# IntptrMax/YoloSharp

Measured on AMD Instinct MI355X. Metric: train images/sec YOLOv8n 640x640 bs=64/GPU, higher is better.
Workload: dtype bf16; 1 GPU; YOLOv8n detect train step (fwd+loss+bwd+AdamW), 64x3x640x640 per GPU, COCO-80 synthetic labels; global_batch=64, parallelism=dp1

## Files before the change

yolosharp_amd/csrc/conv_wgrad.hip:

```cpp
#include "ys_internal.h"
#include "ys_kernels.h"
#include <atomic>
#include <cstdlib>

template <class T, int MRA, int NRB>
__global__ void __launch_bounds__(256)
conv_wgrad_kernel(WgradArgs a) {
  constexpr int EPL = Elem<T>::EPL;
  constexpr int KS = 4 * EPL;
  constexpr int COT = MRA * 16, CIT = NRB * 16;
  constexpr int PD = COT + 16 / (int)sizeof(T);
  constexpr int PX = CIT + 16 / (int)sizeof(T);
  constexpr int STAGE_BYTES = 4 * KS * (PD + PX) * (int)sizeof(T);
  constexpr int RED_BYTES = 4 * COT * CIT * 4;
  constexpr int LDS_BYTES = STAGE_BYTES > RED_BYTES ? STAGE_BYTES : RED_BYTES;
  __shared__ uint4 smem[LDS_BYTES / 16];
  T* sD = (T*)smem;
  T* sX = sD + 4 * KS * PD;

  const int tid = threadIdx.x, lane = tid & 63, wave = tid >> 6, li = lane & 15, q = lane >> 4;
  const int ci_tiles = (a.Cin + CIT - 1) / CIT;
  const int co0 = (blockIdx.y / ci_tiles) * COT;
  const int ci0 = (blockIdx.y % ci_tiles) * CIT;
  const int tap = blockIdx.z;
  const int kh = tap / a.KW, kw = tap % a.KW;
  const int HWo = a.Hout * a.Wout;
  const long steps_total = ((long)a.M + KS - 1) / KS;
  const long steps_per_blk = (steps_total + gridDim.x - 1) / gridDim.x;
  const long sb = (long)blockIdx.x * steps_per_blk;
  long se = sb + steps_per_blk;
  if (se > steps_total) se = steps_total;
  const long iters = (steps_per_blk + 3) / 4;

  f32x4 acc[MRA][NRB];
#pragma unroll
  for (int i = 0; i < MRA; i++)
#pragma unroll
    for (int j = 0; j < NRB; j++) acc[i][j] = f32x4_zero();

  T* myD = sD + wave * KS * PD;
  T* myX = sX + wave * KS * PX;
  const char* dyb = (const char*)a.dy;
  const char* xb = (const char*)a.x;
  constexpr int DV = COT / EPL;
  constexpr int XV = CIT / EPL;

  constexpr int ND = (KS * DV + 63) / 64, NX = (KS * XV + 63) / 64;
  uint4 rd[ND], rx[NX];
  auto fetch = [&](long it) {
    const long step = sb + it * 4 + wave;
    const bool active = step < se;
    const long p0 = step * KS;
#pragma unroll
    for (int k = 0; k < ND; k++) {
      const int v = lane + 64 * k;
      const int pr = v / DV, cv = v % DV;
      const long p = p0 + pr;
      const int c = co0 + cv * EPL;
      uint4 val = ys_zero16();
      if (v < KS * DV && active && p < a.M && c < a.Cout) {
        const long bb = p / HWo;
        const long rr = p - bb * HWo;
        const long drow = a.dy_rh ? bb * a.dy_bstride + (rr / a.Wout) * a.dy_rh + (rr % a.Wout) * a.dy_rw + a.dy_r0
                                  : bb * a.dy_bstride + rr;
        val = ys_ld16(dyb + ((drow * a.dy_ldc) + a.dy_coff + c) * (long)sizeof(T));
      }
      rd[k] = val;
    }
#pragma unroll
    for (int k = 0; k < NX; k++) {
      const int v = lane + 64 * k;
      const int pr = v / XV, cv = v % XV;
      const long p = p0 + pr;
      const int c = ci0 + cv * EPL;
      uint4 val = ys_zero16();
      if (v < KS * XV && active && p < a.M && c < a.Cin) {
        const int b = (int)(p / HWo);
        const int r = (int)(p - (long)b * HWo);
        const int oh = r / a.Wout, ow = r - oh * a.Wout;
        const int ih = oh * a.stride + kh - a.pad, iw = ow * a.stride + kw - a.pad;
        if (ih >= 0 && ih < a.Hin && iw >= 0 && iw < a.Win)
          val = ys_ld16(xb + ((((long)b * a.in_bstride + (long)ih * a.Win + iw) * a.in_ldc) + a.in_coff + c) * (long)sizeof(T));
      }
      rx[k] = val;
    }
  };
  fetch(0);
  for (long it = 0; it < iters; it++) {
#pragma unroll
    for (int k = 0; k < ND; k++) {
      const int v = lane + 64 * k;
      if (v < KS * DV) *(uint4*)(myD + (v / DV) * PD + (v % DV) * EPL) = rd[k];
    }
#pragma unroll
    for (int k = 0; k < NX; k++) {
      const int v = lane + 64 * k;
      if (v < KS * XV) *(uint4*)(myX + (v / XV) * PX + (v % XV) * EPL) = rx[k];
    }
    ys_wave_sync();
    if (it + 1 < iters) fetch(it + 1);
    uint4 fa[MRA], fb[NRB];
#pragma unroll
    for (int i = 0; i < MRA; i++) {
      alignas(16) T tmp[EPL];
#pragma unroll
      for (int e = 0; e < EPL; e++) tmp[e] = myD[(q * EPL + e) * PD + i * 16 + li];
      fa[i] = ys_pack_elems(tmp);
    }
#pragma unroll
    for (int j = 0; j < NRB; j++) {
      alignas(16) T tmp[EPL];
#pragma unroll
      for (int e = 0; e < EPL; e++) tmp[e] = myX[(q * EPL + e) * PX + j * 16 + li];
      fb[j] = ys_pack_elems(tmp);
    }
#pragma unroll
    for (int i = 0; i < MRA; i++)
#pragma unroll
      for (int j = 0; j < NRB; j++) acc[i][j] = ys_mma<T>(fa[i], fb[j], acc[i][j]);
    ys_wave_sync();
  }
  __syncthreads();
  float* sR = (float*)smem;
#pragma unroll
  for (int i = 0; i < MRA; i++)
#pragma unroll
    for (int j = 0; j < NRB; j++)
#pragma unroll
      for (int r = 0; r < 4; r++)
        sR[(wave * COT + i * 16 + 4 * q + r) * CIT + j * 16 + li] = acc[i][j][r];
  __syncthreads();
  float* outp = a.partial + (long)blockIdx.x * a.Cout * a.KH * a.KW * a.Cin;
  for (int e = tid; e < COT * CIT; e += 256) {
    const int co = co0 + e / CIT, ci = ci0 + e % CIT;
    if (co < a.Cout && ci < a.Cin) {
      const float v = sR[e] + sR[COT * CIT + e] + sR[2 * COT * CIT + e] + sR[3 * COT * CIT + e];
      outp[((long)co * a.KH * a.KW + tap) * a.Cin + ci] = v;
    }
  }
}

__global__ void __launch_bounds__(512)
wgrad_reduce_kernel(const float* __restrict__ partial, int splits, long n, int cin_pad, int cin_real,
                    float* __restrict__ grad) {
  __shared__ float sred[16][32];
  const int o = threadIdx.x & 31, sl = threadIdx.x >> 5;
  const long i = (long)blockIdx.x * 32 + o;
  float gprev = 0.f; long gidx = -1;
  if (sl == 0 && i < n) {
    const long row = i / cin_pad;
    const int ci = (int)(i - row * cin_pad);
    if (ci < cin_real) { gidx = row * cin_real + ci; gprev = grad[gidx]; }
  }
  float s0 = 0.f, s1 = 0.f, s2 = 0.f, s3 = 0.f;
  if (i < n) {
    int k = sl;
    for (; k + 48 < splits; k += 64) {
      s0 += partial[(long)k * n + i];
      s1 += partial[(long)(k + 16) * n + i];
      s2 += partial[(long)(k + 32) * n + i];
      s3 += partial[(long)(k + 48) * n + i];
    }
    for (; k < splits; k += 16) s0 += partial[(long)k * n + i];
  }
  sred[sl][o] = (s0 + s1) + (s2 + s3);
  __syncthreads();
  if (gidx >= 0) {
    float t = 0.f;
#pragma unroll
    for (int w = 0; w < 16; w++) t += sred[w][o];
    grad[gidx] = gprev + t;
  }
}

__device__ __forceinline__ unsigned wg_uniform(unsigned v) {
#ifdef YS_EMU_BUILD
  return v;
#else
  return (unsigned)__builtin_amdgcn_readfirstlane((int)v);
#endif
}
#define YS_WG_TWO_MAX 2
template <int MRA, int NRB, int TAPS>
__global__ void __launch_bounds__(TAPS == 9 ? 576 : 256, (TAPS == 9 && MRA * NRB <= YS_WG_TWO_MAX) ? 5 : 1)
conv_wgrad_tr_kernel(WgradArgs a) {
  constexpr int NT = TAPS == 9 ? 576 : 256;
  constexpr int NW = NT / 64;
  constexpr int COT = MRA * 16, CIT = NRB * 16;
  constexpr int DV = COT / 8, XV = CIT / 8;
  constexpr int TPMAX = TAPS == 9 ? 256 : 128;
  constexpr int ND = (TPMAX * DV + NT - 1) / NT;
  constexpr int NX = TAPS == 9 ? 5 : (TPMAX * XV + NT - 1) / NT;
  YS_DYN_LDS(lds);
  const int tid = threadIdx.x, lane = tid & 63, wave = tid >> 6, li = lane & 15, q = lane >> 4;
  const int TW = 1 << a.TWS, TP = a.TH * TW;
  const int nkb = (TP + 31) >> 5;
  const int ZR = nkb * 32;
  char* sDb = (char*)lds;
  const int ci_tiles = (a.Cin + CIT - 1) / CIT;
  const int co0 = (blockIdx.y / ci_tiles) * COT;
  const int ci0 = (blockIdx.y % ci_tiles) * CIT;
  const char* dyb = (const char*)a.dy;
  const char* xb = (const char*)a.x;
  const int S = a.stride;
  const int npatch = a.PH * a.PW * XV;

  for (int i = tid; i < a.pdb / 4; i += NT) ((unsigned*)(sDb + (size_t)ZR * a.pdb))[i] = 0u;

  const ys_rsrcv_t rsD = ys_make_rsrcv(dyb + (long)a.dy_coff * 2L, a.dybytes);
  const ys_rsrcv_t rsX = ys_make_rsrcv(xb + (long)a.in_coff * 2L, a.xbytes);
  uint4 rd[ND], rx[NX];
  constexpr unsigned YS_WG_NOUNIT = 0xffffffffu;
  unsigned doff[ND], drc[ND], dlds[ND], xoff[NX], xrc[NX], xlds[NX];
#pragma unroll
  for (int k = 0; k < ND; k++) {
    const int idx = tid + NT * k;
    const int p = idx / DV, u = idx - p * DV;
    const int ty = p >> a.TWS, tx = p & (TW - 1);
    const int c = co0 + u * 8;
    const bool slot = idx < TP * DV;
    doff[k] = (((unsigned)ty * (unsigned)a.Wout + (unsigned)tx) * (unsigned)a.dy_ldc + (unsigned)c) * 2u;
    drc[k] = (slot && c < a.Cout) ? ((unsigned)ty << 16 | (unsigned)tx) : YS_WG_NOUNIT;
    dlds[k] = slot ? (unsigned)(p * a.pdb + u * 16) : YS_WG_NOUNIT;
#ifndef YS_EMU_BUILD
    asm volatile("" : "+v"(doff[k]), "+v"(drc[k]), "+v"(dlds[k]));
#endif
  }
#pragma unroll
  for (int k = 0; k < NX; k++) {
    const int idx = tid + NT * k;
    const int pix = idx / XV, u = idx - pix * XV;
    const int r = pix / a.PW, cc = pix - r * a.PW;
    const int c = ci0 + u * 8;
    const bool slot = idx < npatch;
    xoff[k] = (((unsigned)r * (unsigned)a.Win + (unsigned)cc) * (unsigned)a.in_ldc + (unsigned)c) * 2u;
    xrc[k] = (slot && c < a.Cin) ? ((unsigned)r << 16 | (unsigned)cc) : YS_WG_NOUNIT;
    xlds[k] = slot ? (unsigned)((ZR + 1) * a.pdb + pix * a.pxb + u * 16) : YS_WG_NOUNIT;
#ifndef YS_EMU_BUILD
    asm volatile("" : "+v"(xoff[k]), "+v"(xrc[k]), "+v"(xlds[k]));
#endif
  }
  auto fetch = [&](int txi, int tyi, int b) {
    const int oy0 = tyi * a.TH, ox0 = txi * TW;
    const unsigned dh = (unsigned)((a.Hout - oy0) < a.TH ? (a.Hout - oy0) : a.TH), dw = (unsigned)((a.Wout - ox0) < TW ? (a.Wout - ox0) : TW);
    const unsigned dorg = wg_uniform((((unsigned)b * (unsigned)a.dy_bstride + (unsigned)oy0 * (unsigned)a.Wout + (unsigned)ox0) * (unsigned)a.dy_ldc) * 2u);
#pragma unroll
    for (int k = 0; k < ND; k++) {
      const bool ok = (bool)((int)((drc[k] >> 16) < dh) & (int)((drc[k] & 0xffffu) < dw));
      rd[k] = ys_bufld16(rsD, ok ? dorg + doff[k] : YS_BUF_OOB);
    }
    const int iy0 = oy0 * S - a.pad, ix0 = ox0 * S - a.pad;
    const unsigned rlo = iy0 < 0 ? (unsigned)-iy0 : 0u, clo = ix0 < 0 ? (unsigned)-ix0 : 0u;
    const unsigned rn = (unsigned)((a.Hin - iy0) < a.PH ? (a.Hin - iy0) : a.PH) - rlo, cn = (unsigned)((a.Win - ix0) < a.PW ? (a.Win - ix0) : a.PW) - clo;
    const unsigned xorg = wg_uniform((((unsigned)b * (unsigned)a.in_bstride + (unsigned)iy0 * (unsigned)a.Win + (unsigned)ix0) * (unsigned)a.in_ldc) * 2u);
#pragma unroll
    for (int k = 0; k < NX; k++) {
      const bool ok = (bool)((int)(((xrc[k] >> 16) - rlo) < rn) & (int)(((xrc[k] & 0xffffu) - clo) < cn));
      rx[k] = ys_bufld16(rsX, ok ? xorg + xoff[k] : YS_BUF_OOB);
    }
  };
  int stx, sty, stb;
  {
    const int G = (int)gridDim.x;
    stx = G % a.tiles_x; const int rem = G / a.tiles_x;
    sty = rem % a.tiles_y; stb = rem / a.tiles_y;
  }
  auto advance = [&](int& txi, int& tyi, int& b) {
    txi += stx; if (txi >= a.tiles_x) { txi -= a.tiles_x; tyi++; }
    tyi += sty; if (tyi >= a.tiles_y) { tyi -= a.tiles_y; b++; }
    b += stb;
  };

  f32x4 acc[MRA][NRB];
#pragma unroll
  for (int i = 0; i < MRA; i++)
#pragma unroll
    for (int j = 0; j < NRB; j++) acc[i][j] = f32x4_zero();

  const int tap = TAPS == 9 ? wave : 0;
  const int kh = tap / 3, kw = tap - kh * 3;
  const int rr = li >> 2, c4 = li & 3;
  unsigned dof[2], xof[2];
  int ty0[2], tx0[2];
#pragma unroll
  for (int h = 0; h < 2; h++) {
    const int p0 = 16 * h + 4 * q + rr;
    ty0[h] = p0 >> a.TWS; tx0[h] = p0 & (TW - 1);
    dof[h] = (unsigned)(p0 * a.pdb + c4 * 8);
    xof[h] = (unsigned)((size_t)(ZR + 1) * a.pdb) + (unsigned)(((ty0[h] * S + kh) * a.PW + tx0[h] * S + kw) * a.pxb + c4 * 8);
  }
  const unsigned dstep = 32u * (unsigned)a.pdb;
  const unsigned xstep = (unsigned)((32 >> a.TWS) * S * a.PW * a.pxb);
  const unsigned zof = (unsigned)(ZR * a.pdb + c4 * 8);
  const unsigned xzero = (unsigned)((ZR + 1) * a.pdb + c4 * 8);
  const int rows_kb = 32 >> a.TWS;
  const char* lb = (const char*)lds;

  int tile = blockIdx.x;
  int txi, tyi, b;
  {
    int t = tile;
    txi = t % a.tiles_x; t /= a.tiles_x;
    tyi = t % a.tiles_y; b = t / a.tiles_y;
  }
  int ntx = txi, nty = tyi, nb = b;
  if (tile < a.ntiles) fetch(txi, tyi, b);
  while (tile < a.ntiles) {
    ys_barrier_lds();
#pragma unroll
    for (int k = 0; k < ND; k++)
      if (dlds[k] != YS_WG_NOUNIT) *(uint4*)((char*)lds + dlds[k]) = rd[k];
#pragma unroll
    for (int k = 0; k < NX; k++)
      if (xlds[k] != YS_WG_NOUNIT) *(uint4*)((char*)lds + xlds[k]) = rx[k];
    ys_barrier_lds();
    const int oy0 = tyi * a.TH, ox0 = txi * TW;
    const int ntile = tile + gridDim.x;
    advance(ntx, nty, nb);
    if (ntile < a.ntiles) fetch(ntx, nty, nb);
    const int tylim = (a.Hout - oy0) < a.TH ? (a.Hout - oy0) : a.TH;
    const bool colok0 = (ox0 + tx0[0]) < a.Wout, colok1 = (ox0 + tx0[1]) < a.Wout;
    for (int kb = (TAPS == 9 ? 0 : wave); kb < nkb; kb += (TAPS == 9 ? 1 : NW)) {
      uint2 ra[2][MRA], rb[2][NRB];
#pragma unroll
      for (int h = 0; h < 2; h++) {
        const int ty = ty0[h] + kb * rows_kb;
        const bool ok = (h == 0 ? colok0 : colok1) && ty < tylim;
        const unsigned d = ok ? dof[h] + (unsigned)kb * dstep : zof;
        const unsigned x = ty < a.TH ? xof[h] + (unsigned)kb * xstep : xzero;
#pragma unroll
        for (int i = 0; i < MRA; i++) ra[h][i] = ys_lds_tr_b64(lb + d + i * 32);
#pragma unroll
        for (int j = 0; j < NRB; j++) rb[h][j] = ys_lds_tr_b64(lb + x + j * 32);
      }
#pragma unroll
      for (int i = 0; i < MRA; i++) ys_lds_tr_wait(ra[0][i], ra[1][i]);
#pragma unroll
      for (int j = 0; j < NRB; j++) ys_lds_tr_wait(rb[0][j], rb[1][j]);
      uint4 fa[MRA], fb[NRB];
#pragma unroll
      for (int i = 0; i < MRA; i++) fa[i] = make_uint4(ra[0][i].x, ra[0][i].y, ra[1][i].x, ra[1][i].y);
#pragma unroll
      for (int j = 0; j < NRB; j++) fb[j] = make_uint4(rb[0][j].x, rb[0][j].y, rb[1][j].x, rb[1][j].y);
#pragma unroll
      for (int i = 0; i < MRA; i++)
#pragma unroll
        for (int j = 0; j < NRB; j++) acc[i][j] = ys_mma<bf16_t>(fa[i], fb[j], acc[i][j]);
    }
    tile = ntile; txi = ntx; tyi = nty;
  }

  float* outp = a.partial + (long)blockIdx.x * a.Cout * a.KH * a.KW * a.Cin;
  const int taps = a.KH * a.KW;
  if (TAPS == 9) {
#pragma unroll
    for (int i = 0; i < MRA; i++)
#pragma unroll
      for (int j = 0; j < NRB; j++)
#pragma unroll
        for (int r = 0; r < 4; r++) {
          const int co = co0 + i * 16 + 4 * q + r, ci = ci0 + j * 16 + li;
          if (co < a.Cout && ci < a.Cin) outp[((long)co * taps + tap) * a.Cin + ci] = acc[i][j][r];
        }
  } else {
    __syncthreads();
    float* sR = (float*)lds;
#pragma unroll
    for (int i = 0; i < MRA; i++)
#pragma unroll
      for (int j = 0; j < NRB; j++)
#pragma unroll
        for (int r = 0; r < 4; r++) sR[(wave * COT + i * 16 + 4 * q + r) * CIT + j * 16 + li] = acc[i][j][r];
    __syncthreads();
    for (int e = tid; e < COT * CIT; e += NT) {
      const int co = co0 + e / CIT, ci = ci0 + e % CIT;
      if (co < a.Cout && ci < a.Cin) {
        float v = 0.f;
        for (int w = 0; w < NW; w++) v += sR[w * COT * CIT + e];
        outp[(long)co * a.Cin + ci] = v;
      }
    }
  }
}

struct WgPlan { int ok, taps9, mra, nrb, th, tws, tx, ty, ph, pw, pdb, pxb, gx; size_t lds; };
static int wg_pitch_bytes(int ch) {
  int s = (ch * 2 + 31) / 32;
  if (!(s & 1)) s++;
  return s * 32;
}
static bool wgrad_view_bytes(const WgradArgs& a, unsigned& dyb, unsigned& xb) {
  const long dpix = (long)(a.B - 1) * a.dy_bstride + (long)a.Hout * a.Wout, xpix = (long)(a.B - 1) * a.in_bstride + (long)a.Hin * a.Win;
  const long d = (dpix * a.dy_ldc - a.dy_coff) * 2L, x = (xpix * a.in_ldc - a.in_coff) * 2L;
  if (d <= 0 || x <= 0 || d >= (1L << 31) || x >= (1L << 31)) return false;
  dyb = (unsigned)d; xb = (unsigned)x;
  return true;
}
#ifdef YS_TRIAGE
static int g_wg_force_th = 0, g_wg_force_tws = 0, g_wg_force_percu = 0;
extern "C" __attribute__((visibility("default"))) int ys_debug_wgrad_force(int th, int tws, int per_cu) { g_wg_force_th = th; g_wg_force_tws = tws; g_wg_force_percu = per_cu; return 0; }
#else
constexpr int g_wg_force_th = 0, g_wg_force_tws = 0, g_wg_force_percu = 0;
#endif
static WgPlan wgrad_tr_plan(const WgradArgs& a) {
  WgPlan p{};
  { unsigned d0, x0; if (!wgrad_view_bytes(a, d0, x0)) return p; }
  const bool k3 = a.KH == 3 && a.KW == 3 && a.pad == 1 && (a.stride == 1 || a.stride == 2);
  const bool k1 = a.KH == 1 && a.KW == 1 && a.pad == 0 && a.stride == 1;
  if (a.dy_rh || !(k3 || k1)) return p;
  const int cof = (a.Cout + 15) / 16, cif = (a.Cin + 15) / 16;
  p.mra = cof >= 4 ? ((cof % 5 == 0) ? 5 : 4) : cof;
  p.nrb = cif >= 4 ? 4 : cif;
  p.taps9 = k3 ? 1 : 0;
  if (k3) {
    static const int ok_pairs[][2] = {{1, 1}, {1, 2}, {1, 3}, {1, 4}, {2, 1}, {2, 2}, {2, 3}, {2, 4}, {3, 1}, {3, 2}, {3, 3}, {3, 4}, {4, 1}, {4, 2}, {5, 1}};
    int best_cost = 1 << 30;
    for (auto& pr : ok_pairs) {
      const int m = pr[0], n = pr[1];
      if (m > cof || n > cif) continue;
      const int cost = ys_cdiv(cof, m) * ys_cdiv(cif, n) * (m + n) * 16 + (ys_cdiv(cof, m) * m - cof) + (ys_cdiv(cif, n) * n - cif) + (n > m ? 1 : 0);
      if (cost < best_cost) { best_cost = cost; p.mra = m; p.nrb = n; }
    }
  }
  const int nt = k3 ? 576 : 256, tpmax = k3 ? 256 : 128;
  const int cot = p.mra * 16, cit = p.nrb * 16, xv = cit / 8;
  const int nxu = (k3 ? 5 : (tpmax * xv + nt - 1) / nt) * nt;
  const int S = a.stride;
  p.pdb = wg_pitch_bytes(cot);
  p.pxb = S == 1 ? wg_pitch_bytes(cit) : ((cit * 2 + 15) / 32) * 32 + 16;
  double best = 1e30;
  for (int tws = 2; tws <= 5; tws++) {
    const int tw = 1 << tws;
    if (tw > a.Wout && tws > 2 && (tw >> 1) >= a.Wout) continue;
    if (g_wg_force_tws && tws != g_wg_force_tws) continue;
    for (int th = 1; th <= a.Hout && th * tw <= tpmax; th++) {
      if (g_wg_force_th && th != g_wg_force_th) continue;
      const int ph = (th - 1) * S + a.KH, pw = (tw - 1) * S + a.KW;
      if (ph * pw * xv > nxu) continue;
      const int nkb = (th * tw + 31) / 32;
      size_t lds = (size_t)(nkb * 32 + 1) * p.pdb + (size_t)ph * pw * p.pxb;
      if (!k3 && lds < (size_t)4 * cot * cit * 4) lds = (size_t)4 * cot * cit * 4;
      if (lds > 150 * 1024) continue;
      const int tx = ys_cdiv(a.Wout, tw), ty = ys_cdiv(a.Hout, th);
      const double cost = (double)tx * ty * ((double)ph * pw * cit + (double)nkb * 32 * cot + 0.5 * nkb * 32 * (cot + cit) + 3000.0);
      if (cost < best) { best = cost; p.ok = 1; p.th = th; p.tws = tws; p.tx = tx; p.ty = ty; p.ph = ph; p.pw = pw; p.lds = lds; }
    }
  }
  if (!p.ok) return p;
  const int gy = ys_cdiv(a.Cout, cot) * ys_cdiv(a.Cin, cit);
  const long ntiles = (long)p.tx * p.ty * a.B;
  int per_cu = (int)((150 * 1024) / p.lds);
  const int per_cu_max = k3 ? (p.mra * p.nrb <= YS_WG_TWO_MAX ? 2 : 1) : 4;
  if (per_cu > per_cu_max) per_cu = per_cu_max;
  if (g_wg_force_percu && g_wg_force_percu < per_cu) per_cu = g_wg_force_percu;
  if (per_cu < 1) per_cu = 1;
  long gx = ((long)ys_cu_count() * per_cu) / gy;
  gx = gx / 8 * 8;
  if (gx < 8) gx = 8;
  const long wsmax = (48L << 20) / ((long)a.Cout * a.KH * a.KW * a.Cin * 4);
  if (gx > wsmax) gx = wsmax > 0 ? wsmax : 1;
  if (gx > ntiles) gx = ntiles;
  const long per = (ntiles + gx - 1) / gx;
  gx = (ntiles + per - 1) / per;
  p.gx = (int)gx;
  return p;
}

template <int MRA, int NRB, int TAPS>
static void wgrad_tr_launch_t(hipStream_t st, WgradArgs a, const WgPlan& p) {
  a.TH = p.th; a.TWS = p.tws; a.tiles_x = p.tx; a.tiles_y = p.ty; a.ntiles = p.tx * p.ty * a.B;
  wgrad_view_bytes(a, a.dybytes, a.xbytes);
  a.PH = p.ph; a.PW = p.pw; a.pdb = p.pdb; a.pxb = p.pxb;
  const int gy = ys_cdiv(a.Cout, MRA * 16) * ys_cdiv(a.Cin, NRB * 16);
  static std::atomic<unsigned> attr_done{0};
  int dev_id = 0;
  (void)hipGetDevice(&dev_id);
  if (!(attr_done.load(std::memory_order_relaxed) & (1u << (dev_id & 31)))) {
    hipFuncSetAttribute((const void*)conv_wgrad_tr_kernel<MRA, NRB, TAPS>, hipFuncAttributeMaxDynamicSharedMemorySize, 160 * 1024);
    attr_done.fetch_or(1u << (dev_id & 31), std::memory_order_relaxed);
  }
  char lab[160] = "";
  if (ys_kprof_enabled()) snprintf(lab, sizeof(lab), "wgrad_tr k%d s%d cin%d cout%d M%d tile%dx%d grid%dx%d lds%d", a.KH, a.stride, a.Cin, a.Cout, a.M, p.th, 1 << p.tws, p.gx, gy, (int)p.lds);
  YsKprofScope prof(st, "conv_wgrad", lab);
  YS_LAUNCH_LDS((conv_wgrad_tr_kernel<MRA, NRB, TAPS>), dim3(p.gx, gy), (TAPS == 9 ? 576 : 256), p.lds, st, a);
}

static bool wgrad_tr_dispatch(hipStream_t st, const WgradArgs& a, const WgPlan& p) {
#define WT(M_, N_) if (p.mra == M_ && p.nrb == N_) { if (p.taps9) wgrad_tr_launch_t<M_, N_, 9>(st, a, p); else wgrad_tr_launch_t<M_, N_, 1>(st, a, p); return true; }
  WT(1, 1) WT(1, 2) WT(1, 3) WT(1, 4)
  WT(2, 1) WT(2, 2) WT(2, 3) WT(2, 4)
  WT(3, 1) WT(3, 2) WT(3, 3) WT(3, 4)
  WT(4, 1) WT(4, 2) WT(4, 3) WT(4, 4)
  WT(5, 1) WT(5, 2) WT(5, 3) WT(5, 4)
#undef WT
  return false;
}

template <class T, int MRA, int NRB>
static void wgrad_launch_t(hipStream_t st, const WgradArgs& a, int splits) {
  const int co_tiles = ys_cdiv(a.Cout, MRA * 16), ci_tiles = ys_cdiv(a.Cin, NRB * 16);
  dim3 grid(splits, co_tiles * ci_tiles, a.KH * a.KW);
  char lab[128] = "";
  if (ys_kprof_enabled()) snprintf(lab, sizeof(lab), "wgrad k%d s%d cin%d cout%d M%d splits%d tiles%d", a.KH, a.stride, a.Cin, a.Cout, a.M, splits, co_tiles * ci_tiles);
  YsKprofScope prof(st, "conv_wgrad", lab);
  YS_LAUNCH((conv_wgrad_kernel<T, MRA, NRB>), grid, 256, st, a);
}

template <class T>
static void wgrad_dispatch(hipStream_t st, const WgradArgs& a, int splits) {
  const int cof = (a.Cout + 15) / 16, cif = (a.Cin + 15) / 16;
  const int mra = cof >= 4 ? ((cof % 5 == 0) ? 5 : 4) : cof;
  const int nrb = cif >= 4 ? 4 : cif;
#define WG(M_, N_) if (mra == M_ && nrb == N_) { wgrad_launch_t<T, M_, N_>(st, a, splits); return; }
  WG(1, 1) WG(1, 2) WG(1, 3) WG(1, 4)
  WG(2, 1) WG(2, 2) WG(2, 3) WG(2, 4)
  WG(3, 1) WG(3, 2) WG(3, 3) WG(3, 4)
  WG(4, 1) WG(4, 2) WG(4, 3) WG(4, 4)
  WG(5, 1) WG(5, 2) WG(5, 3) WG(5, 4)
#undef WG
}

int ys_wgrad_splits(const WgradArgs& a, int dtype) {
  if (dtype == YS_BF16) {
    const int gs = ys_wgrad_gemm_splits(a);
    if (gs) return gs;
    const WgPlan p = wgrad_tr_plan(a);
    if (p.ok) return p.gx;
  }
  const int ks = dtype == YS_BF16 ? 32 : 16;
  const int cof = (a.Cout + 15) / 16, cif = (a.Cin + 15) / 16;
  const int mra = cof >= 4 ? ((cof % 5 == 0) ? 5 : 4) : cof;
  const int nrb = cif >= 4 ? 4 : cif;
  const long tiles = (long)ys_cdiv(a.Cout, mra * 16) * ys_cdiv(a.Cin, nrb * 16) * a.KH * a.KW;
  const long steps = ((long)a.M + ks - 1) / ks;
  long s = (2048 + tiles - 1) / tiles;
  const long smax = (steps + 15) / 16;
  if (s > smax) s = smax;
  if (s < 1) s = 1;
  if (s > 128) s = 128;
  return (int)s;
}

int ys_wgrad_launch(hipStream_t st, int dtype, const WgradArgs& a, int splits, int cin_real, float* grad, int* used_splits) {
  const int epl = dtype == YS_BF16 ? 8 : 4;
  if (a.Cin % epl || a.in_ldc % epl || a.in_coff % epl || a.dy_ldc % epl || a.dy_coff % epl) {
    ys_set_error("wgrad: channel counts/strides must be multiples of %d (Cin %d Cout %d)", epl, a.Cin, a.Cout);
    return YS_ERR_INVALID_ARG;
  }
  bool done = false;
  if (dtype == YS_BF16) {
    const int used = ys_wgrad_gemm_launch(st, a, splits);
    if (used) { splits = used; done = true; }
  }
  if (dtype == YS_BF16 && !done) {
    WgPlan p = wgrad_tr_plan(a);
    if (p.ok) {
      if (splits < p.gx) p.gx = splits;
      splits = p.gx;
      done = wgrad_tr_dispatch(st, a, p);
    }
  }
  if (!done) {
    if (dtype == YS_BF16) wgrad_dispatch<bf16_t>(st, a, splits);
    else wgrad_dispatch<float>(st, a, splits);
  }
  const long n = (long)a.Cout * a.KH * a.KW * a.Cin;
  if (used_splits) { *used_splits = splits; return YS_OK; }
  YS_LAUNCH(wgrad_reduce_kernel, ys_cdiv(n, 32), 512, st, (const float*)a.partial, splits, n, a.Cin, cin_real, grad);
  return YS_OK;
}

__global__ void __launch_bounds__(512)
wgrad_reduce_batched_kernel(const WgRedDesc* __restrict__ descs, int nd) {
  constexpr int NSUB = YS_WGRED_OUT_PER_BLOCK / 128;
  __shared__ float4 sred[NSUB][16][32];
  int lo = 0, hi = nd - 1;
  const long blk = blockIdx.x;
  while (lo < hi) { const int mid = (lo + hi + 1) >> 1; if (descs[mid].blk0 <= blk) lo = mid; else hi = mid - 1; }
  const WgRedDesc d = descs[lo];
  const float* __restrict__ partial = d.partial;
  const int splits = d.splits;
  const long n = d.n;
  const int o = threadIdx.x & 31, sl = threadIdx.x >> 5;
  const long i0 = (blk - d.blk0) * YS_WGRED_OUT_PER_BLOCK + o * 4;
  auto add4 = [](float4& acc, const float4& v) { acc.x += v.x; acc.y += v.y; acc.z += v.z; acc.w += v.w; };
  float4 tot[NSUB];
  if (splits <= 16) {
    float4 v[NSUB];
#pragma unroll
    for (int u = 0; u < NSUB; u++) {
      const long i = i0 + u * 128;
      v[u] = (i < n && sl < splits) ? *(const float4*)(partial + (long)sl * n + i) : make_float4(0.f, 0.f, 0.f, 0.f);
    }
#pragma unroll
    for (int u = 0; u < NSUB; u++) tot[u] = make_float4((v[u].x + 0.f) + (0.f + 0.f), (v[u].y + 0.f) + (0.f + 0.f), (v[u].z + 0.f) + (0.f + 0.f), (v[u].w + 0.f) + (0.f + 0.f));
  } else {
#pragma unroll
    for (int u = 0; u < NSUB; u++) {
      const long i = i0 + u * 128;
      float4 s0 = make_float4(0.f, 0.f, 0.f, 0.f), s1 = s0, s2 = s0, s3 = s0;
      if (i < n) {
        int k = sl;
        for (; k + 48 < splits; k += 64) {
          const float4 v0 = *(const float4*)(partial + (long)k * n + i);
          const float4 v1 = *(const float4*)(partial + (long)(k + 16) * n + i);
          const float4 v2 = *(const float4*)(partial + (long)(k + 32) * n + i);
          const float4 v3 = *(const float4*)(partial + (long)(k + 48) * n + i);
          add4(s0, v0); add4(s1, v1); add4(s2, v2); add4(s3, v3);
        }
        for (; k < splits; k += 16) add4(s0, *(const float4*)(partial + (long)k * n + i));
      }
      tot[u] = make_float4((s0.x + s1.x) + (s2.x + s3.x), (s0.y + s1.y) + (s2.y + s3.y), (s0.z + s1.z) + (s2.z + s3.z), (s0.w + s1.w) + (s2.w + s3.w));
    }
  }
#pragma unroll
  for (int u = 0; u < NSUB; u++) sred[u][sl][o] = tot[u];
  __syncthreads();
  if (sl < NSUB) {
    const long i = i0 + sl * 128;
    if (i < n) {
      const long row = i / d.cin_pad;
      const int ci = (int)(i - row * d.cin_pad);
      int nreal = d.cin_real - ci; if (nreal > 4) nreal = 4;
      if (nreal > 0) {
        const long gidx = row * d.cin_real + ci;
        float4 t = make_float4(0.f, 0.f, 0.f, 0.f);
#pragma unroll
        for (int w = 0; w < 16; w++) add4(t, sred[sl][w][o]);
        const float tv[4] = {t.x, t.y, t.z, t.w};
#pragma unroll
        for (int e = 0; e < 4; e++) if (e < nreal) d.grad[gidx + e] = d.grad[gidx + e] + tv[e];
      }
    }
  }
}
int ys_wgrad_reduce_batched_launch(hipStream_t st, const WgRedDesc* descs_dev, int n_desc, long total_blocks) {
  if (n_desc <= 0 || total_blocks <= 0) return YS_OK;
  YS_LAUNCH(wgrad_reduce_batched_kernel, (int)total_blocks, 512, st, descs_dev, n_desc);
  return YS_OK;
}

template <class T>
__global__ void __launch_bounds__(256)
weight_prep_kernel(const float* __restrict__ w, int Cout, int taps, int cin_real, int cin_pad, int cout_pad,
                   T* __restrict__ wf, T* __restrict__ wd, int phase) {
  const long i = (long)blockIdx.x * blockDim.x + threadIdx.x;
  const long nf = (long)Cout * taps * cin_pad;
  if (i < nf) {
    const int ci = (int)(i % cin_pad);
    const long r = i / cin_pad;
    wf[i] = Elem<T>::from_f(ci < cin_real ? w[r * cin_real + ci] : 0.f);
  }
  if (wd) {
    const long nd = (long)cin_real * taps * cout_pad;
    if (i < nd) {
      int co, ci, tap;
      if (phase) {
        ys_phase_wd_index(i, cin_real, cout_pad, ci, tap, co);
      } else {
        co = (int)(i % cout_pad);
        const long r = i / cout_pad;
        const int tapf = (int)(r % taps);
        ci = (int)(r / taps);
        tap = taps - 1 - tapf;
      }
      wd[i] = Elem<T>::from_f(co < Cout ? w[((long)co * taps + tap) * cin_real + ci] : 0.f);
    }
  }
}

int ys_weight_prep_launch(hipStream_t st, int dtype, const float* w, int Cout, int taps, int cin_real, int cin_pad,
                          int cout_pad, void* wf, void* wd, int phase) {
  const long nf = (long)Cout * taps * cin_pad;
  const long nd = wd ? (long)cin_real * taps * cout_pad : 0;
  const long n = nf > nd ? nf : nd;
  if (dtype == YS_BF16)
    YS_LAUNCH((weight_prep_kernel<bf16_t>), ys_cdiv(n, 256), 256, st, w, Cout, taps, cin_real, cin_pad, cout_pad, (bf16_t*)wf, (bf16_t*)wd, phase);
  else
    YS_LAUNCH((weight_prep_kernel<float>), ys_cdiv(n, 256), 256, st, w, Cout, taps, cin_real, cin_pad, cout_pad, (float*)wf, (float*)wd, phase);
  return YS_OK;
}
```

Before: 7695 images/s.

## Add multi-stage LDS ring with direct buffer-to-LDS loads for 3x3 wgrad

For 3x3 weight-gradient kernels where each block handles at least two tiles, the old register-staged fetch (global to VGPR, then store to LDS) is replaced by an N-stage LDS ring. The ring is filled with buffer loads that write straight into LDS, and a dynamic vmcnt wait lets the next tile's loads overlap the MFMA work on the current tile. This aims to hide global-load latency and cut VGPR pressure and LDS store instructions. It costs extra LDS per block, which can lower occupancy, and it drops some large taps9 tile combinations (4x3, 4x4, 5x2 and up) from dispatch.

```diff
diff --git a/yolosharp_amd/csrc/conv_wgrad.hip b/yolosharp_amd/csrc/conv_wgrad.hip
--- a/yolosharp_amd/csrc/conv_wgrad.hip
+++ b/yolosharp_amd/csrc/conv_wgrad.hip
@@ -181,36 +181,216 @@
 #endif
 }
 #define YS_WG_TWO_MAX 2
-template <int MRA, int NRB, int TAPS>
+struct WgRing {
+  int ns;
+  int kd, kx;
+  int nrd, nrx;
+  unsigned stage;
+};
+constexpr int wg_pitch_bytes(int ch) {
+  int s = (ch * 2 + 31) / 32;
+  if (!(s & 1)) s++;
+  return s * 32;
+}
+constexpr int wg_pitch_s2_bytes(int ch) { return ((ch * 2 + 15) / 32) * 32 + 16; }
+constexpr int wg_nx(int nrb, bool k3) { return k3 ? 5 : (128 * nrb * 2 + 255) / 256; }
+constexpr int wg_kdmax(int mra) { return ((257 * wg_pitch_bytes(mra * 16) + 1023) / 1024 + 8) / 9; }
+constexpr int wg_kxmax(int nrb) {
+  const int pix = wg_nx(nrb, true) * 576 / (nrb * 2);
+  const int pb = wg_pitch_s2_bytes(nrb * 16) > wg_pitch_bytes(nrb * 16) ? wg_pitch_s2_bytes(nrb * 16) : wg_pitch_bytes(nrb * 16);
+  return ((pix * pb + 1023) / 1024 + 8) / 9;
+}
+template <int MRA, int NRB, int TAPS, bool RING>
 __global__ void __launch_bounds__(TAPS == 9 ? 576 : 256, (TAPS == 9 && MRA * NRB <= YS_WG_TWO_MAX) ? 5 : 1)
-conv_wgrad_tr_kernel(WgradArgs a) {
+conv_wgrad_tr_kernel(WgradArgs a, WgRing rg) {
   constexpr int NT = TAPS == 9 ? 576 : 256;
   constexpr int NW = NT / 64;
   constexpr int COT = MRA * 16, CIT = NRB * 16;
   constexpr int DV = COT / 8, XV = CIT / 8;
   constexpr int TPMAX = TAPS == 9 ? 256 : 128;
-  constexpr int ND = (TPMAX * DV + NT - 1) / NT;
-  constexpr int NX = TAPS == 9 ? 5 : (TPMAX * XV + NT - 1) / NT;
   YS_DYN_LDS(lds);
   const int tid = threadIdx.x, lane = tid & 63, wave = tid >> 6, li = lane & 15, q = lane >> 4;
   const int TW = 1 << a.TWS, TP = a.TH * TW;
   const int nkb = (TP + 31) >> 5;
   const int ZR = nkb * 32;
-  char* sDb = (char*)lds;
+  const unsigned xbase = RING ? (unsigned)rg.nrd * 1024u : (unsigned)((ZR + 1) * a.pdb);
   const int ci_tiles = (a.Cin + CIT - 1) / CIT;
   const int co0 = (blockIdx.y / ci_tiles) * COT;
   const int ci0 = (blockIdx.y % ci_tiles) * CIT;
   const char* dyb = (const char*)a.dy;
   const char* xb = (const char*)a.x;
   const int S = a.stride;
+  constexpr unsigned YS_WG_NOUNIT = 0xffffffffu;
+
+  int stx, sty, stb;
+  {
+    const int G = (int)gridDim.x;
+    stx = G % a.tiles_x; const int rem = G / a.tiles_x;
+    sty = rem % a.tiles_y; stb = rem / a.tiles_y;
+  }
+  auto advance = [&](int& txi, int& tyi, int& b) {
+    txi += stx; if (txi >= a.tiles_x) { txi -= a.tiles_x; tyi++; }
+    tyi += sty; if (tyi >= a.tiles_y) { tyi -= a.tiles_y; b++; }
+    b += stb;
+  };
+
+  f32x4 acc[MRA][NRB];
+#pragma unroll
+  for (int i = 0; i < MRA; i++)
+#pragma unroll
+    for (int j = 0; j < NRB; j++) acc[i][j] = f32x4_zero();
+
+  const int tap = TAPS == 9 ? wave : 0;
+  const int kh = tap / 3, kw = tap - kh * 3;
+  const int rr = li >> 2, c4 = li & 3;
+  unsigned dof[2], xof[2];
+  int ty0[2], tx0[2];
+#pragma unroll
+  for (int h = 0; h < 2; h++) {
+    const int p0 = 16 * h + 4 * q + rr;
+    ty0[h] = p0 >> a.TWS; tx0[h] = p0 & (TW - 1);
+    dof[h] = (unsigned)(p0 * a.pdb + c4 * 8);
+    xof[h] = xbase + (unsigned)(((ty0[h] * S + kh) * a.PW + tx0[h] * S + kw) * a.pxb + c4 * 8);
+  }
+  const unsigned dstep = 32u * (unsigned)a.pdb;
+  const unsigned xstep = (unsigned)((32 >> a.TWS) * S * a.PW * a.pxb);
+  const unsigned zof = (unsigned)(ZR * a.pdb + c4 * 8);
+  const unsigned xzero = xbase + (unsigned)(c4 * 8);
+  const int rows_kb = 32 >> a.TWS;
+  auto multiply = [&](const char* lb, int txi, int tyi) {
+    const int oy0 = tyi * a.TH, ox0 = txi * TW;
+    const int tylim = (a.Hout - oy0) < a.TH ? (a.Hout - oy0) : a.TH;
+    const bool colok0 = (ox0 + tx0[0]) < a.Wout, colok1 = (ox0 + tx0[1]) < a.Wout;
+    for (int kb = (TAPS == 9 ? 0 : wave); kb < nkb; kb += (TAPS == 9 ? 1 : NW)) {
+      uint2 ra[2][MRA], rb[2][NRB];
+#pragma unroll
+      for (int h = 0; h < 2; h++) {
+        const int ty = ty0[h] + kb * rows_kb;
+        const bool ok = (h == 0 ? colok0 : colok1) && ty < tylim;
+        const unsigned d = ok ? dof[h] + (unsigned)kb * dstep : zof;
+        const unsigned x = ty < a.TH ? xof[h] + (unsigned)kb * xstep : xzero;
+#pragma unroll
+        for (int i = 0; i < MRA; i++) ra[h][i] = ys_lds_tr_b64(lb + d + i * 32);
+#pragma unroll
+        for (int j = 0; j < NRB; j++) rb[h][j] = ys_lds_tr_b64(lb + x + j * 32);
+      }
+#pragma unroll
+      for (int i = 0; i < MRA; i++) ys_lds_tr_wait(ra[0][i], ra[1][i]);
+#pragma unroll
+      for (int j = 0; j < NRB; j++) ys_lds_tr_wait(rb[0][j], rb[1][j]);
+      uint4 fa[MRA], fb[NRB];
+#pragma unroll
+      for (int i = 0; i < MRA; i++) fa[i] = make_uint4(ra[0][i].x, ra[0][i].y, ra[1][i].x, ra[1][i].y);
+#pragma unroll
+      for (int j = 0; j < NRB; j++) fb[j] = make_uint4(rb[0][j].x, rb[0][j].y, rb[1][j].x, rb[1][j].y);
+#pragma unroll
+      for (int i = 0; i < MRA; i++)
+#pragma unroll
+        for (int j = 0; j < NRB; j++) acc[i][j] = ys_mma<bf16_t>(fa[i], fb[j], acc[i][j]);
+    }
+  };
+
+  int tile = blockIdx.x;
+  int txi, tyi, b;
+  {
+    int t = tile;
+    txi = t % a.tiles_x; t /= a.tiles_x;
+    tyi = t % a.tiles_y; b = t / a.tiles_y;
+  }
+  int ntx = txi, nty = tyi, nb = b;
+
+  if constexpr (RING) {
+  static_assert(TAPS == 9, "the 4-wave 1x1 launches keep the register fetch (wgrad_tr_plan)");
+  constexpr int KDMAX = wg_kdmax(MRA), KXMAX = wg_kxmax(NRB);
+  const ys_rsrc_t rsD = ys_make_rsrc(dyb + (long)a.dy_coff * 2L, a.dybytes);
+  const ys_rsrc_t rsX = ys_make_rsrc(xb + (long)a.in_coff * 2L, a.xbytes);
+  const unsigned wv = wg_uniform((unsigned)wave);
+  const unsigned spare = (unsigned)(rg.nrd + rg.nrx);
+  unsigned doff[KDMAX], drc[KDMAX], xoff[KXMAX], xrc[KXMAX];
+#pragma unroll
+  for (int k = 0; k < KDMAX; k++) {
+    doff[k] = 0u; drc[k] = YS_WG_NOUNIT;
+    if (k < rg.kd) {
+      const unsigned byte = (wv + (unsigned)(NW * k)) * 1024u + (unsigned)lane * 16u;
+      const unsigned p = byte / (unsigned)a.pdb, u = (byte - p * (unsigned)a.pdb) >> 4;
+      const unsigned ty = p >> a.TWS, tx = p & (unsigned)(TW - 1);
+      const int c = co0 + (int)u * 8;
+      doff[k] = ((ty * (unsigned)a.Wout + tx) * (unsigned)a.dy_ldc + (unsigned)c) * 2u;
+      if (p < (unsigned)TP && u < (unsigned)DV && c < a.Cout) drc[k] = ty << 16 | tx;
+    }
+#ifndef YS_EMU_BUILD
+    asm volatile("" : "+v"(doff[k]), "+v"(drc[k]));
+#endif
+  }
+#pragma unroll
+  for (int k = 0; k < KXMAX; k++) {
+    xoff[k] = 0u; xrc[k] = YS_WG_NOUNIT;
+    if (k < rg.kx) {
+      const unsigned byte = (wv + (unsigned)(NW * k)) * 1024u + (unsigned)lane * 16u;
+      const unsigned pix = byte / (unsigned)a.pxb, u = (byte - pix * (unsigned)a.pxb) >> 4;
+      const unsigned r = pix / (unsigned)a.PW, cc = pix - r * (unsigned)a.PW;
+      const int c = ci0 + (int)u * 8;
+      xoff[k] = ((r * (unsigned)a.Win + cc) * (unsigned)a.in_ldc + (unsigned)c) * 2u;
+      if (pix < (unsigned)(a.PH * a.PW) && u < (unsigned)XV && c < a.Cin) xrc[k] = r << 16 | cc;
+    }
+#ifndef YS_EMU_BUILD
+    asm volatile("" : "+v"(xoff[k]), "+v"(xrc[k]));
+#endif
+  }
+  auto request = [&](int txi, int tyi, int b, char* sb) {
+    const int oy0 = tyi * a.TH, ox0 = txi * TW;
+    const unsigned dh = (unsigned)((a.Hout - oy0) < a.TH ? (a.Hout - oy0) : a.TH), dw = (unsigned)((a.Wout - ox0) < TW ? (a.Wout - ox0) : TW);
+    const unsigned dorg = wg_uniform((((unsigned)b * (unsigned)a.dy_bstride + (unsigned)oy0 * (unsigned)a.Wout + (unsigned)ox0) * (unsigned)a.dy_ldc) * 2u);
+#pragma unroll
+    for (int k = 0; k < KDMAX; k++)
+      if (k < rg.kd) {
+        const bool ok = (bool)((int)((drc[k] >> 16) < dh) & (int)((drc[k] & 0xffffu) < dw));
+        const unsigned rq = wv + (unsigned)(NW * k);
+        ys_bufld_lds16_nom0(rsD, ok ? dorg + doff[k] : YS_BUF_OOB, 0u, sb + (rq < (unsigned)rg.nrd ? rq : spare) * 1024u);
+      }
+    const int iy0 = oy0 * S - a.pad, ix0 = ox0 * S - a.pad;
+    const unsigned rlo = iy0 < 0 ? (unsigned)-iy0 : 0u, clo = ix0 < 0 ? (unsigned)-ix0 : 0u;
+    const unsigned rn = (unsigned)((a.Hin - iy0) < a.PH ? (a.Hin - iy0) : a.PH) - rlo, cn = (unsigned)((a.Win - ix0) < a.PW ? (a.Win - ix0) : a.PW) - clo;
+    const unsigned xorg = wg_uniform((((unsigned)b * (unsigned)a.in_bstride + (unsigned)iy0 * (unsigned)a.Win + (unsigned)ix0) * (unsigned)a.in_ldc) * 2u);
+#pragma unroll
+    for (int k = 0; k < KXMAX; k++)
+      if (k < rg.kx) {
+        const bool ok = (bool)((int)(((xrc[k] >> 16) - rlo) < rn) & (int)(((xrc[k] & 0xffffu) - clo) < cn));
+        const unsigned rq = wv + (unsigned)(NW * k);
+        ys_bufld_lds16_nom0(rsX, ok ? xorg + xoff[k] : YS_BUF_OOB, 0u, sb + (rq < (unsigned)rg.nrx ? (unsigned)rg.nrd + rq : spare) * 1024u);
+      }
+  };
+  const int G = (int)gridDim.x;
+  const int nper = rg.kd + rg.kx;
+  char* const lb0 = (char*)lds;
+  unsigned cst = 0u, fst = 0u;
+  int ftile = tile;
+#pragma unroll 1
+  for (int j = 0; j < rg.ns - 1; j++) {
+    if (ftile < a.ntiles) request(ntx, nty, nb, lb0 + fst);
+    ftile += G; advance(ntx, nty, nb);
+    fst += rg.stage;
+  }
+  while (tile < a.ntiles) {
+    if (rg.ns == 3 && tile + G < a.ntiles) ys_wait_vm_dyn(nper); else ys_wait_vm<0>();
+    ys_barrier_lds();
+    if (ftile < a.ntiles) request(ntx, nty, nb, lb0 + fst);
+    ftile += G; advance(ntx, nty, nb);
+    fst += rg.stage; if (fst == (unsigned)rg.ns * rg.stage) fst = 0u;
+    multiply(lb0 + cst, txi, tyi);
+    tile += G; advance(txi, tyi, b);
+    cst += rg.stage; if (cst == (unsigned)rg.ns * rg.stage) cst = 0u;
+  }
+  } else {
+  constexpr int ND = (TPMAX * DV + NT - 1) / NT;
+  constexpr int NX = wg_nx(NRB, TAPS == 9);
   const int npatch = a.PH * a.PW * XV;
-
+  char* sDb = (char*)lds;
   for (int i = tid; i < a.pdb / 4; i += NT) ((unsigned*)(sDb + (size_t)ZR * a.pdb))[i] = 0u;
 
   const ys_rsrcv_t rsD = ys_make_rsrcv(dyb + (long)a.dy_coff * 2L, a.dybytes);
   const ys_rsrcv_t rsX = ys_make_rsrcv(xb + (long)a.in_coff * 2L, a.xbytes);
   uint4 rd[ND], rx[NX];
-  constexpr unsigned YS_WG_NOUNIT = 0xffffffffu;
   unsigned doff[ND], drc[ND], dlds[ND], xoff[NX], xrc[NX], xlds[NX];
 #pragma unroll
   for (int k = 0; k < ND; k++) {
@@ -259,51 +439,6 @@
       rx[k] = ys_bufld16(rsX, ok ? xorg + xoff[k] : YS_BUF_OOB);
     }
   };
-  int stx, sty, stb;
-  {
-    const int G = (int)gridDim.x;
-    stx = G % a.tiles_x; const int rem = G / a.tiles_x;
-    sty = rem % a.tiles_y; stb = rem / a.tiles_y;
-  }
-  auto advance = [&](int& txi, int& tyi, int& b) {
-    txi += stx; if (txi >= a.tiles_x) { txi -= a.tiles_x; tyi++; }
-    tyi += sty; if (tyi >= a.tiles_y) { tyi -= a.tiles_y; b++; }
-    b += stb;
-  };
-
-  f32x4 acc[MRA][NRB];
-#pragma unroll
-  for (int i = 0; i < MRA; i++)
-#pragma unroll
-    for (int j = 0; j < NRB; j++) acc[i][j] = f32x4_zero();
-
-  const int tap = TAPS == 9 ? wave : 0;
-  const int kh = tap / 3, kw = tap - kh * 3;
-  const int rr = li >> 2, c4 = li & 3;
-  unsigned dof[2], xof[2];
-  int ty0[2], tx0[2];
-#pragma unroll
-  for (int h = 0; h < 2; h++) {
-    const int p0 = 16 * h + 4 * q + rr;
-    ty0[h] = p0 >> a.TWS; tx0[h] = p0 & (TW - 1);
-    dof[h] = (unsigned)(p0 * a.pdb + c4 * 8);
-    xof[h] = (unsigned)((size_t)(ZR + 1) * a.pdb) + (unsigned)(((ty0[h] * S + kh) * a.PW + tx0[h] * S + kw) * a.pxb + c4 * 8);
-  }
-  const unsigned dstep = 32u * (unsigned)a.pdb;
-  const unsigned xstep = (unsigned)((32 >> a.TWS) * S * a.PW * a.pxb);
-  const unsigned zof = (unsigned)(ZR * a.pdb + c4 * 8);
-  const unsigned xzero = (unsigned)((ZR + 1) * a.pdb + c4 * 8);
-  const int rows_kb = 32 >> a.TWS;
-  const char* lb = (const char*)lds;
-
-  int tile = blockIdx.x;
-  int txi, tyi, b;
-  {
-    int t = tile;
-    txi = t % a.tiles_x; t /= a.tiles_x;
-    tyi = t % a.tiles_y; b = t / a.tiles_y;
-  }
-  int ntx = txi, nty = tyi, nb = b;
   if (tile < a.ntiles) fetch(txi, tyi, b);
   while (tile < a.ntiles) {
     ys_barrier_lds();
@@ -314,40 +449,12 @@
     for (int k = 0; k < NX; k++)
       if (xlds[k] != YS_WG_NOUNIT) *(uint4*)((char*)lds + xlds[k]) = rx[k];
     ys_barrier_lds();
-    const int oy0 = tyi * a.TH, ox0 = txi * TW;
     const int ntile = tile + gridDim.x;
     advance(ntx, nty, nb);
     if (ntile < a.ntiles) fetch(ntx, nty, nb);
-    const int tylim = (a.Hout - oy0) < a.TH ? (a.Hout - oy0) : a.TH;
-    const bool colok0 = (ox0 + tx0[0]) < a.Wout, colok1 = (ox0 + tx0[1]) < a.Wout;
-    for (int kb = (TAPS == 9 ? 0 : wave); kb < nkb; kb += (TAPS == 9 ? 1 : NW)) {
-      uint2 ra[2][MRA], rb[2][NRB];
-#pragma unroll
-      for (int h = 0; h < 2; h++) {
-        const int ty = ty0[h] + kb * rows_kb;
-        const bool ok = (h == 0 ? colok0 : colok1) && ty < tylim;
-        const unsigned d = ok ? dof[h] + (unsigned)kb * dstep : zof;
-        const unsigned x = ty < a.TH ? xof[h] + (unsigned)kb * xstep : xzero;
-#pragma unroll
-        for (int i = 0; i < MRA; i++) ra[h][i] = ys_lds_tr_b64(lb + d + i * 32);
-#pragma unroll
-        for (int j = 0; j < NRB; j++) rb[h][j] = ys_lds_tr_b64(lb + x + j * 32);
-      }
-#pragma unroll
-      for (int i = 0; i < MRA; i++) ys_lds_tr_wait(ra[0][i], ra[1][i]);
-#pragma unroll
-      for (int j = 0; j < NRB; j++) ys_lds_tr_wait(rb[0][j], rb[1][j]);
-      uint4 fa[MRA], fb[NRB];
-#pragma unroll
-      for (int i = 0; i < MRA; i++) fa[i] = make_uint4(ra[0][i].x, ra[0][i].y, ra[1][i].x, ra[1][i].y);
-#pragma unroll
-      for (int j = 0; j < NRB; j++) fb[j] = make_uint4(rb[0][j].x, rb[0][j].y, rb[1][j].x, rb[1][j].y);
-#pragma unroll
-      for (int i = 0; i < MRA; i++)
-#pragma unroll
-        for (int j = 0; j < NRB; j++) acc[i][j] = ys_mma<bf16_t>(fa[i], fb[j], acc[i][j]);
-    }
+    multiply((const char*)lds, txi, tyi);
     tile = ntile; txi = ntx; tyi = nty;
+  }
   }
 
   float* outp = a.partial + (long)blockIdx.x * a.Cout * a.KH * a.KW * a.Cin;
@@ -383,12 +490,10 @@
   }
 }
 
-struct WgPlan { int ok, taps9, mra, nrb, th, tws, tx, ty, ph, pw, pdb, pxb, gx; size_t lds; };
-static int wg_pitch_bytes(int ch) {
-  int s = (ch * 2 + 31) / 32;
-  if (!(s & 1)) s++;
-  return s * 32;
-}
+struct WgPlan { int ok, taps9, mra, nrb, th, tws, tx, ty, ph, pw, pdb, pxb, gx, ns; size_t lds; WgRing ring; };
+#ifndef YS_WG_RING_MAX
+#define YS_WG_RING_MAX 2
+#endif
 static bool wgrad_view_bytes(const WgradArgs& a, unsigned& dyb, unsigned& xb) {
   const long dpix = (long)(a.B - 1) * a.dy_bstride + (long)a.Hout * a.Wout, xpix = (long)(a.B - 1) * a.in_bstride + (long)a.Hin * a.Win;
   const long d = (dpix * a.dy_ldc - a.dy_coff) * 2L, x = (xpix * a.in_ldc - a.in_coff) * 2L;
@@ -424,10 +529,10 @@
   }
   const int nt = k3 ? 576 : 256, tpmax = k3 ? 256 : 128;
   const int cot = p.mra * 16, cit = p.nrb * 16, xv = cit / 8;
-  const int nxu = (k3 ? 5 : (tpmax * xv + nt - 1) / nt) * nt;
+  const int nxu = wg_nx(p.nrb, k3) * nt;
   const int S = a.stride;
   p.pdb = wg_pitch_bytes(cot);
-  p.pxb = S == 1 ? wg_pitch_bytes(cit) : ((cit * 2 + 15) / 32) * 32 + 16;
+  p.pxb = S == 1 ? wg_pitch_bytes(cit) : wg_pitch_s2_bytes(cit);
   double best = 1e30;
   for (int tws = 2; tws <= 5; tws++) {
     const int tw = 1 << tws;
@@ -463,10 +568,27 @@
   const long per = (ntiles + gx - 1) / gx;
   gx = (ntiles + per - 1) / per;
   p.gx = (int)gx;
+  p.ns = 1;
+  if (k3 && per >= 2) {
+    const int nw = nt / 64, nkb = (p.th * (1 << p.tws) + 31) / 32;
+    WgRing r{};
+    r.nrd = ys_cdiv((nkb * 32 + 1) * p.pdb, 1024); r.nrx = ys_cdiv(p.ph * p.pw * p.pxb, 1024);
+    r.kd = ys_cdiv(r.nrd, nw); r.kx = ys_cdiv(r.nrx, nw);
+    const int fillers = r.kd * nw - r.nrd + r.kx * nw - r.nrx;
+    r.stage = (unsigned)(r.nrd + r.nrx + (fillers ? 1 : 0)) * 1024u;
+    if (r.kd <= wg_kdmax(p.mra) && r.kx <= wg_kxmax(p.nrb))
+      for (int ns = YS_WG_RING_MAX; ns >= 2; ns--) {
+        const size_t lds = (size_t)ns * r.stage;
+        if (lds * per_cu > 150 * 1024) continue;
+        if (ns == 3 && r.kd + r.kx > 15) continue;
+        r.ns = ns; p.ns = ns; p.lds = lds; p.ring = r;
+        break;
+      }
+  }
   return p;
 }
 
-template <int MRA, int NRB, int TAPS>
+template <int MRA, int NRB, int TAPS, bool RING>
 static void wgrad_tr_launch_t(hipStream_t st, WgradArgs a, const WgPlan& p) {
   a.TH = p.th; a.TWS = p.tws; a.tiles_x = p.tx; a.tiles_y = p.ty; a.ntiles = p.tx * p.ty * a.B;
   wgrad_view_bytes(a, a.dybytes, a.xbytes);
@@ -476,17 +598,30 @@
   int dev_id = 0;
   (void)hipGetDevice(&dev_id);
   if (!(attr_done.load(std::memory_order_relaxed) & (1u << (dev_id & 31)))) {
-    hipFuncSetAttribute((const void*)conv_wgrad_tr_kernel<MRA, NRB, TAPS>, hipFuncAttributeMaxDynamicSharedMemorySize, 160 * 1024);
+    hipFuncSetAttribute((const void*)conv_wgrad_tr_kernel<MRA, NRB, TAPS, RING>, hipFuncAttributeMaxDynamicSharedMemorySize, 160 * 1024);
     attr_done.fetch_or(1u << (dev_id & 31), std::memory_order_relaxed);
   }
   char lab[160] = "";
-  if (ys_kprof_enabled()) snprintf(lab, sizeof(lab), "wgrad_tr k%d s%d cin%d cout%d M%d tile%dx%d grid%dx%d lds%d", a.KH, a.stride, a.Cin, a.Cout, a.M, p.th, 1 << p.tws, p.gx, gy, (int)p.lds);
+  if (ys_kprof_enabled()) {
+    const int n = snprintf(lab, sizeof(lab), "wgrad_tr k%d s%d cin%d cout%d M%d tile%dx%d grid%dx%d lds%d", a.KH, a.stride, a.Cin, a.Cout, a.M, p.th, 1 << p.tws, p.gx, gy, (int)p.lds);
+    if (RING && n > 0 && n < (int)sizeof(lab)) snprintf(lab + n, sizeof(lab) - n, " ring%d", p.ns);
+  }
   YsKprofScope prof(st, "conv_wgrad", lab);
-  YS_LAUNCH_LDS((conv_wgrad_tr_kernel<MRA, NRB, TAPS>), dim3(p.gx, gy), (TAPS == 9 ? 576 : 256), p.lds, st, a);
+  YS_LAUNCH_LDS((conv_wgrad_tr_kernel<MRA, NRB, TAPS, RING>), dim3(p.gx, gy), (TAPS == 9 ? 576 : 256), p.lds, st, a, p.ring);
 }
 
 static bool wgrad_tr_dispatch(hipStream_t st, const WgradArgs& a, const WgPlan& p) {
-#define WT(M_, N_) if (p.mra == M_ && p.nrb == N_) { if (p.taps9) wgrad_tr_launch_t<M_, N_, 9>(st, a, p); else wgrad_tr_launch_t<M_, N_, 1>(st, a, p); return true; }
+#define WT(M_, N_) if (p.mra == M_ && p.nrb == N_) { if (p.ns > 1) wgrad_tr_launch_t<M_, N_, 9, true>(st, a, p); else wgrad_tr_launch_t<M_, N_, 9, false>(st, a, p); return true; }
+  if (p.taps9) {
+    WT(1, 1) WT(1, 2) WT(1, 3) WT(1, 4)
+    WT(2, 1) WT(2, 2) WT(2, 3) WT(2, 4)
+    WT(3, 1) WT(3, 2) WT(3, 3) WT(3, 4)
+    WT(4, 1) WT(4, 2)
+    WT(5, 1)
+    return false;
+  }
+#undef WT
+#define WT(M_, N_) if (p.mra == M_ && p.nrb == N_) { wgrad_tr_launch_t<M_, N_, 1, false>(st, a, p); return true; }
   WT(1, 1) WT(1, 2) WT(1, 3) WT(1, 4)
   WT(2, 1) WT(2, 2) WT(2, 3) WT(2, 4)
   WT(3, 1) WT(3, 2) WT(3, 3) WT(3, 4)
```

Measured after the change: 7810 images/s (median of 6 runs). +1.5%, better.
